# tomershay100/mp3-steganography-lib

Hardware: AMD Instinct MI355X
Metric: MP3 frames/sec (decode+re-encode) @44.1kHz stereo 128kbps, 1→8 GPU (higher is better)
Workload: dtype f64 (decode) / int32 (encode); 1 GPU; 10000-frame full decode->stego-embed->re-encode pipeline per MI355X (BASELINE configs[2]); MP3 main data + side info resident in HBM, MP3 frames out; the message cursor chain is decided and the serial chains of the rate loop are checked on the device inside every step; frames_per_gpu=10000, channels=2, message_bits=536, chain_verdict_units_to_redo=0, message_variant_entries=1874, parallelism=frames sharded over 1 GPU(s), no collective

## Files before the change

mp3-steganography-lib_amd/csrc/k_rate.hpp:

```cpp
#pragma once
#ifndef MP3S_RL_STATS
#define MP3S_RL_STATS 0
#endif
#ifndef MP3S_RL_OCC
#define MP3S_RL_OCC 6
#endif
#if MP3S_RL_STATS
__device__ unsigned long long g_rl_stats[128];
extern "C" __attribute__((visibility("default"))) int mp3s_debug_rl_stats(unsigned long long *out, int clear)
{
    (void)hipDeviceSynchronize();
    int rc = (int)hipMemcpyFromSymbol(out, HIP_SYMBOL(g_rl_stats), sizeof(unsigned long long) * 128);
    if (clear) { unsigned long long z[128] = {}; rc |= (int)hipMemcpyToSymbol(HIP_SYMBOL(g_rl_stats), z, sizeof z); }
    return rc;
}
#define RL_STAT(i, v) do { if ((threadIdx.x & 63) == 0) atomicAdd(&g_rl_stats[(i)], (unsigned long long)(v)); } while (0)
#define RL_CLK() __builtin_readcyclecounter()
#else
#define RL_STAT(i, v) do { } while (0)
#endif

namespace mp3s {

__device__ __forceinline__ uint32_t mulr_u(uint32_t a, uint32_t b) { return (uint32_t)(((uint64_t)a * b + 0x80000000ull) >> 32); }

constexpr int REDO_CAP = 4096, REDO_HEAD = 4, REDO_WORDS = REDO_HEAD + 6 * REDO_CAP;
constexpr int REDO_GROUPS = 256;
constexpr int REDO_CHAIN_MAX = 64;
constexpr int RL_WAVES = 4;
constexpr int RL_NP = 5;

struct RlTables {
    uint16_t int2idx[10000];
    uint2 hl[256];
    uint32_t c1w[16];
    uint8_t transform[64];
    uint32_t subdiv[292];
};

__device__ __forceinline__ int lin_bits_of(int t)
{
    return t < 16 ? 0 : (int)(((t < 24 ? 0xDA864321u : 0xDB987654u) >> (4 * (t & 7))) & 15u);
}

struct RlState {
    int big_values, count1, c1sel, r0c, r1c, a1, a2, a3, ts0, ts1, ts2;
    bool addr_fresh, used_addr_in;
};

__device__ __forceinline__ int family_of(int t) { return t == 13 ? 0 : (t == 15 ? 1 : (t < 24 ? 2 : 3)); }

__device__ __forceinline__ uint32_t pair_bits(const RlTables &tb, int fam, int lb, int x, int y)
{
    const int xx = x > 14 ? 15 : x, yy = y > 14 ? 15 : y;
    const uint32_t h = tb.hl[xx * 16 + yy].x;
    return ((h >> (5 * fam)) & 31u) + ((h >> 20) & 3u) + (uint32_t)lb * ((h >> 22) & 3u);
}
__device__ __forceinline__ int sel3(int r, int a, int b, int c) { return r == 0 ? a : (r == 1 ? b : c); }

__device__ __forceinline__ uint32_t rl_scale_of(int step)
{
    return (uint32_t)c_tab.steptabi[(step + 127) & 127];
}

__device__ __forceinline__ int rl_quantize(const RlTables &tb, const uint32_t (&xa)[2 * RL_NP], int32_t (&ix)[2 * RL_NP],
                                           int step, uint32_t scalei, uint32_t xrmax)
{
    const int idx = step + 127;
    if (idx < 0 || idx > 127) return -1;
    const uint32_t lnmax = mulr_u(xrmax, scalei);
    if (lnmax > 165140u) return 16384;
    if (lnmax < 10000u) {
#pragma unroll
        for (int e = 0; e < 2 * RL_NP; e++) ix[e] = tb.int2idx[mulr_u(xa[e], scalei)];
        return 0;
    }
    const double scale = c_tab.steptab[idx];
    bool big = false;
#pragma unroll
    for (int e = 0; e < 2 * RL_NP; e++) {
        uint32_t a = xa[e];
        asm volatile("" : "+v"(a));
        const uint32_t ln = mulr_u(a, scalei);
        const double dbl = (double)a * scale * 4.656612875e-10;
        const int32_t v = (int32_t)__dsqrt_rn(__dsqrt_rn(dbl) * dbl);
        ix[e] = ln >= 10000u ? v : (int32_t)tb.int2idx[ln < 10000u ? ln : 9999u];
        big |= ix[e] > 8192;
    }
    return __ballot(big) ? 8193 : 0;
}

__device__ __forceinline__ void rl_run_lengths(const RlTables &tb, int k0, int k1, RlState &st)
{
    const unsigned long long nzm = __ballot(k0 != 0), bgm = __ballot(k1 != 0);
    const int L0 = 63 - (nzm ? __builtin_clzll(nzm) : 0), L1 = 63 - (bgm ? __builtin_clzll(bgm) : 0);
    const int r0 = __builtin_amdgcn_readlane(k0, L0), r1 = __builtin_amdgcn_readlane(k1, L1);
    const int P0 = nzm ? 5 * L0 + r0 - 1 : -1, P1 = bgm ? 5 * L1 + r1 - 1 : -1;
    const int count1 = (P0 - P1) >> 1;
    const int bv = (P0 + 1) - 2 * count1;
    st.count1 = count1;
    st.big_values = bv;
    if (bv == 0) {
        st.r0c = 0; st.r1c = 0;
        if (!st.addr_fresh) st.used_addr_in = true;
    } else {
        const uint32_t e = (uint32_t)__builtin_amdgcn_readfirstlane((int)tb.subdiv[bv < 289 ? bv : 288]);
        st.r0c = (int)(e & 15); st.r1c = (int)((e >> 4) & 7);
        st.a1 = (int)((e >> 8) & 1023); st.a2 = (int)((e >> 18) & 1023);
        st.a3 = 2 * bv;
        st.addr_fresh = true;
    }
}

__device__ __forceinline__ int rl_precheck(const RlTables &tb, const uint32_t (&xa)[2 * RL_NP], int p0, RlState &st, int step, uint32_t scalei,
                                           uint32_t xrmax, int limit, bool &q_early)
{
    q_early = false;
    const int idx = step + 127;
    if (idx < 0 || idx > 127) return -1;
    if (mulr_u(xrmax, scalei) > 165140u) { q_early = true; return 100000; }
    const uint32_t t1 = (uint32_t)c_tab.rl_t1[idx], t2 = (uint32_t)c_tab.rl_t2[idx], t8 = (uint32_t)c_tab.rl_t8[idx];
    if (xrmax >= t8) return 100000;
    int k0 = 0, k1 = 0;
    uint32_t nnz = 0, nzp = 0;
#pragma unroll
    for (int m = 0; m < RL_NP; m++) {
        const uint32_t pm = max(xa[2 * m], xa[2 * m + 1]);
        k0 = pm >= t1 ? m + 1 : k0;
        k1 = pm >= t2 ? m + 1 : k1;
        nzp |= pm >= t1 ? 1u << m : 0u;
        nnz += (xa[2 * m] >= t1 ? 1u : 0u) + (xa[2 * m + 1] >= t1 ? 1u : 0u);
    }
    rl_run_lengths(tb, k0, k1, st);
    const int below = min(max(st.big_values - p0, 0), RL_NP);
    nnz += (uint32_t)__builtin_popcount(nzp & ((1u << below) - 1u));
    const int lb = (int)wave_add_u32(nnz) + st.count1;
    return lb >= limit ? lb : -1;
}

__device__ __forceinline__ int rl_body(const RlTables &tb, const int32_t (&ix)[2 * RL_NP], int p0,
                                       RlState &st, const uint8_t *__restrict__ hide, int n_hide, int cursor,
                                       int limit, bool ub_ok, bool &full)
{
    int k0 = 0, k1 = 0;
#pragma unroll
    for (int m = 0; m < RL_NP; m++) {
        const uint32_t o = (uint32_t)(ix[2 * m] | ix[2 * m + 1]);
        k0 = o != 0 ? m + 1 : k0;
        k1 = o > 1 ? m + 1 : k1;
    }
    rl_run_lengths(tb, k0, k1, st);
    const int count1 = st.count1, bv = st.big_values, bvr = 2 * bv;

    uint32_t h[RL_NP], c2[RL_NP + 1];
    uint32_t bnd = 0, acc = 0;
    {
        const int reach = st.a2 > bvr ? st.a2 : bvr;
        const int d_bv = bv - p0, d_reach = ((reach + 1) >> 1) - p0;
#pragma unroll
        for (int m = 0; m < RL_NP; m++) {
            const int x = ix[2 * m], y = ix[2 * m + 1];
            const uint2 hh = tb.hl[(x > 14 ? 15 : x) * 16 + (y > 14 ? 15 : y)];
            h[m] = hh.x;
            bnd += m < d_bv ? hh.y : (m < d_reach ? hh.y & 0xffff0000u : 0u);
        }
        if (count1 > 0) {
#pragma unroll
            for (int m = 0; m < RL_NP; m++) c2[m] = (uint32_t)(ix[2 * m] + 2 * ix[2 * m + 1]);
            c2[RL_NP] = (uint32_t)__builtin_amdgcn_update_dpp(0, (int)c2[0], 0x130, 0xf, 0xf, false);
            const uint32_t c1n = (uint32_t)(2 * count1);
            const uint32_t rel0 = (uint32_t)(p0 - bv);
            const uint32_t keep_even = (rel0 & 1u) ? 0xffff0000u : 0xffffffffu, keep_odd = (rel0 & 1u) ? 0xffffffffu : 0xffff0000u;
#pragma unroll
            for (int m = 0; m < RL_NP; m++) {
                const uint32_t quad = tb.c1w[(c2[m] | (c2[m + 1] << 2)) & 15u];
                acc += rel0 + (uint32_t)m < c1n ? quad & ((m & 1) ? keep_odd : keep_even) : 0u;
            }
            wave_add2(bnd, acc);
        } else bnd = wave_add_u32(bnd);
    }
    const int signs = (int)(acc >> 16), sum0 = signs + (int)(acc & 0xffff), sum1 = signs + 4 * count1;
    int bits;
    if (sum0 < sum1) { st.c1sel = 0; bits = sum0; } else { st.c1sel = 1; bits = sum1; }
    full = false;
    {
        const int lb = bits + (int)(bnd & 0xffffu), ub = bits + (int)(bnd >> 16);
        if (lb >= limit) return lb;
        if (ub_ok && ub < limit) return ub;
        full = true;
    }

    const int a1 = st.a1, a2 = st.a2;
    uint32_t mx0 = 0, mx1 = 0, mx2 = 0;
    int rid[RL_NP];
    const int d_a1 = ((a1 + 1) >> 1) - p0, d_a2 = ((a2 + 1) >> 1) - p0, d_bv3 = bv - p0;
#pragma unroll
    for (int m = 0; m < RL_NP; m++) {
        const uint32_t pm = (uint32_t)max(ix[2 * m], ix[2 * m + 1]);
        const bool in0 = m < d_a1, in1 = !in0 && m < d_a2, in2 = !in0 && !in1 && m < d_bv3;
        mx0 = max(mx0, in0 ? pm : 0u);
        mx1 = max(mx1, in1 ? pm : 0u);
        mx2 = max(mx2, in2 ? pm : 0u);
        rid[m] = in0 ? 0 : (in1 ? 1 : (in2 ? 2 : -1));
    }
    wave_max3(mx0, mx1, mx2);
    const int rmax[3] = {(int)mx0, (int)mx1, (int)mx2};

    int tA[3], tB[3];
    uint32_t Kr[3];
#pragma unroll
    for (int r = 0; r < 3; r++) {
        const int mxr = rmax[r];
        const int need = mxr - 15;
        const int nb = need > 0 ? 32 - __builtin_clz((unsigned)need) : 0;
        const int kA = (int)((0x77766554432100ull >> (4 * nb)) & 15ull);
        const int kB = (int)((0x77665432100000ull >> (4 * nb)) & 15ull);
        const bool none = mxr == 0, small = mxr < 15, esc0 = need == 0;
        tA[r] = none ? 0 : (small ? 13 : (esc0 ? 15 : 16 + kA));
        tB[r] = none ? 0 : (small ? 15 : 24 + kB);
        const uint32_t lbA = (0xDA864321u >> (4 * kA)) & 15u, lbB = (0xDB987654u >> (4 * kB)) & 15u;
        const uint32_t big = (esc0 ? 5u : (10u | (lbA << 16))) | (15u << 8) | (lbB << 20);
        Kr[r] = none ? (25u | (25u << 8)) : (small ? (0u | (5u << 8)) : big);
    }
#if MP3S_RL_STATS
    RL_STAT(63, 1);
    if (rmax[0] < 15 && rmax[1] < 15 && rmax[2] < 15) RL_STAT(64, 1);
    if (rmax[1] < 15 && rmax[2] < 15) RL_STAT(65, 1);
#endif
    uint32_t w0 = 0, w1 = 0, w2 = 0;
#pragma unroll
    for (int m = 0; m < RL_NP; m++) {
        const int r = rid[m];
        const uint32_t kp = (uint32_t)sel3(r, (int)Kr[0], (int)Kr[1], (int)Kr[2]);
        const uint32_t nz = __builtin_amdgcn_ubfe(h[m], 20, 2), esc = __builtin_amdgcn_ubfe(h[m], 22, 2);
        const uint32_t a = __builtin_amdgcn_ubfe(h[m], kp & 31u, 5) + nz + __builtin_amdgcn_ubfe(kp, 16, 4) * esc;
        const uint32_t b = __builtin_amdgcn_ubfe(h[m], (kp >> 8) & 31u, 5) + nz + __builtin_amdgcn_ubfe(kp, 20, 4) * esc;
        const uint32_t v = a | (b << 16);
        w0 += r == 0 ? v : 0u;
        w1 += r == 1 ? v : 0u;
        w2 += r == 2 ? v : 0u;
    }
    wave_add3(w0, w1, w2);
    const uint32_t wsum[3] = {w0, w1, w2};
    int ts[3], rbits[3];
    bool redo[3];
    int idx = cursor;
#pragma unroll
    for (int r = 0; r < 3; r++) {
        ts[r] = 0; rbits[r] = 0; redo[r] = false;
        if (tA[r]) {
            const uint32_t s = wsum[r];
            const int bA = (int)(s & 0xffff), bB = (int)(s >> 16);
            int choice;
            if (tA[r] == 13) choice = (bB <= bA) ? 15 : 13;
            else choice = (bB < bA) ? tB[r] : tA[r];
            if (n_hide > 0 && idx < n_hide) choice = tb.transform[choice * 2 + (hide[idx] & 1)];
            ts[r] = choice;
            if (choice == tA[r]) rbits[r] = bA;
            else if (choice == tB[r]) rbits[r] = bB;
            else redo[r] = true;
            if (choice > 0) idx += 1;
        }
    }
    if (redo[0] || redo[1] || redo[2]) {
        uint32_t extra = 0;
        const int f0 = family_of(ts[0]), f1 = family_of(ts[1]), f2 = family_of(ts[2]);
        const int l0 = lin_bits_of(ts[0]), l1 = lin_bits_of(ts[1]), l2 = lin_bits_of(ts[2]);
#pragma unroll
        for (int m = 0; m < RL_NP; m++) {
            const int r = rid[m];
            const bool rd = r >= 0 && sel3(r, redo[0], redo[1], redo[2]) != 0;
            const uint32_t v = pair_bits(tb, sel3(r, f0, f1, f2), sel3(r, l0, l1, l2), ix[2 * m], ix[2 * m + 1]);
            extra += rd ? v : 0u;
        }
        bits += (int)wave_add_u32(extra);
    }
    st.ts0 = ts[0]; st.ts1 = ts[1]; st.ts2 = ts[2];
    return bits + rbits[0] + rbits[1] + rbits[2];
}

struct RateVariants {
    const int32_t *unit, *cursor;
    int n;
    int16_t *ix; mp3s_gr_out *out; int32_t *en;
    uint8_t *tables;
};

template <bool CHAIN = false>
__device__ __forceinline__ void rate_units(
    const int32_t *__restrict__ mdct, const mp3s_rate_frame *__restrict__ frames, int n_units,
    const uint8_t *__restrict__ hide, int n_hide_all, const int32_t *__restrict__ cursor_in,
    const int32_t *__restrict__ state_in, const int32_t *__restrict__ unit_list, int n_list,
    int16_t *__restrict__ ix_out, mp3s_gr_out *__restrict__ out, int32_t *__restrict__ en_out, int out_base, int compact,
    RateVariants var, const int32_t *__restrict__ cursor_all = nullptr)
{
    const int n_total = n_list + var.n;
    __shared__ __attribute__((aligned(16))) RlTables tb;
#if MP3S_RL_STATS
    const unsigned long long clk0 = RL_CLK();
#endif
    const int sr0 = frames[0].sr_idx;
    const int sr_wg = sr0 >= 0 && sr0 < 3 ? sr0 : 0;
    const int wave = __builtin_amdgcn_readfirstlane(threadIdx.x >> 6), lane = threadIdx.x & 63;
    const int p0 = 5 * lane;
    int2 xpre[RL_NP];
    int u_pre = -1;
    if (!CHAIN) {
        const int li = blockIdx.x * RL_WAVES + wave;
        if (li < n_list + var.n) {
            const int32_t *ul = li >= n_list ? var.unit : unit_list;
            const int lj = li >= n_list ? li - n_list : li;
            u_pre = __builtin_amdgcn_readfirstlane(ul ? ul[lj] : lj);
            if (u_pre >= 0 && u_pre < n_units) {
                const int32_t *xr = mdct + (long)u_pre * 576;
#pragma unroll
                for (int m = 0; m < RL_NP; m++) {
                    xpre[m] = make_int2(0, 0);
                    if (p0 + m < 288) xpre[m] = *reinterpret_cast<const int2 *>(xr + 2 * (p0 + m));
                }
            }
        }
    }
    static_assert(sizeof(tb.int2idx) % 16 == 0 && sizeof(c_tab.int2idx) == sizeof(tb.int2idx), "int2idx is staged 16 bytes at a time");
    static_assert(sizeof(tb.hl) == sizeof(c_tab.rl_hl) && sizeof(tb.hl) % 1024 == 0, "the pair words are staged one wave-load (1 KB) at a time");
    static_assert(offsetof(RlTables, hl) % 16 == 0 && offsetof(RlTables, subdiv) % 16 == 0 && sizeof(tb.subdiv) % 16 == 0, "16-byte pieces in LDS");
    constexpr int I2I_CHUNKS = (int)(sizeof(tb.int2idx) / 16), I2I_ROUNDS = (I2I_CHUNKS + RL_WAVES * 64 - 1) / (RL_WAVES * 64);
    constexpr int HL_CHUNKS = (int)(sizeof(tb.hl) / 16), SD_CHUNKS = (int)(sizeof(tb.subdiv) / 16);
    static_assert(HL_CHUNKS + SD_CHUNKS <= RL_WAVES * 64 && HL_CHUNKS % 64 == 0, "pair words and region table: one piece per thread");
    uint32_t t_c1w = 0, t_tr = 0;
    {
        typedef const __attribute__((address_space(1))) void *gsrc;
        typedef __attribute__((address_space(3))) void *ldst;
        char *const lds0 = reinterpret_cast<char *>(&tb);
        const char *const g_i2i = reinterpret_cast<const char *>(c_tab.int2idx);
#pragma unroll
        for (int r = 0; r < I2I_ROUNDS; r++) {
            const int base = (r * RL_WAVES + wave) * 64;
            if (base + lane < I2I_CHUNKS)
                __builtin_amdgcn_global_load_lds((gsrc)(g_i2i + (size_t)(base + lane) * 16), (ldst)(lds0 + offsetof(RlTables, int2idx) + base * 16), 16, 0, 0);
        }
        {
            const int base = wave * 64;
            const bool is_hl = base < HL_CHUNKS;
            const char *src = is_hl ? reinterpret_cast<const char *>(c_tab.rl_hl) + (size_t)(base + lane) * 16
                                    : reinterpret_cast<const char *>(c_tab.subdiv_lut[sr_wg]) + (size_t)(base - HL_CHUNKS + lane) * 16;
            char *dst = is_hl ? lds0 + offsetof(RlTables, hl) + base * 16 : lds0 + offsetof(RlTables, subdiv) + (base - HL_CHUNKS) * 16;
            if (is_hl || base - HL_CHUNKS + lane < SD_CHUNKS) __builtin_amdgcn_global_load_lds((gsrc)src, (ldst)dst, 16, 0, 0);
        }
        if (threadIdx.x < 16) t_c1w = c_tab.rl_c1w[threadIdx.x];
        if (threadIdx.x < 64) t_tr = c_tab.transform[threadIdx.x >> 1][threadIdx.x & 1];
    }
    auto tables_in = [&]() {
        if (threadIdx.x < 16) tb.c1w[threadIdx.x] = t_c1w;
        if (threadIdx.x < 64) tb.transform[threadIdx.x] = (uint8_t)t_tr;
        __builtin_amdgcn_s_waitcnt(0);
        __syncthreads();
    };
    if (CHAIN) tables_in();

    int li0 = blockIdx.x * RL_WAVES + wave;
    if (li0 >= n_total) { if (!CHAIN) tables_in(); return; }
    do {
    int li = li0;
    uint8_t *tables_out = nullptr;
    if (li >= n_list) {
        li -= n_list;
        tables_out = var.tables;
        unit_list = var.unit; cursor_in = var.cursor; state_in = nullptr;
        ix_out = var.ix; out = var.out; en_out = var.en;
        compact = 2;
    }
    int u = CHAIN ? __builtin_amdgcn_readfirstlane(unit_list ? unit_list[li] : li) : u_pre;
    if (u < 0 || u >= n_units) { if (CHAIN) continue; tables_in(); return; }
    bool chained = false;
    int ch_cursor = 0, ch_state[4] = {0, 0, 0, 0};
    for (int steps = 0; ; steps++) {
    if (CHAIN) __builtin_amdgcn_wave_barrier();
    const mp3s_rate_frame fr = frames[u >> 2];
    const int sr = sr_wg;
    const int max_bits = fr.max_bits;
    const int ci = compact ? li : u;
    const int cursor = chained ? ch_cursor : ((n_hide_all > 0 && cursor_in) ? cursor_in[ci] : 0);
    const int n_hide = min(n_hide_all, fr.hide_end);

    const int32_t *xr = mdct + (long)u * 576;
    uint32_t xa[2 * RL_NP];
    uint32_t negmask = 0, lmax = 0, esum = 0;
    uint32_t pk[2 * RL_NP - 1];
#pragma unroll
    for (int m = 0; m < RL_NP; m++) {
        const int p = p0 + m;
        int2 v = make_int2(0, 0);
        if (!CHAIN) v = xpre[m];
        else if (p < 288) v = *reinterpret_cast<const int2 *>(xr + 2 * p);
        const int32_t vv[2] = {v.x, v.y};
#pragma unroll
        for (int e = 0; e < 2; e++) {
            const uint32_t a = vv[e] < 0 ? (0u - (uint32_t)vv[e]) : (uint32_t)vv[e];
            xa[2 * m + e] = a;
            if (vv[e] < 0) negmask |= 1u << (2 * m + e);
            lmax = max(lmax, a);
            const int32_t sq = (int32_t)(((uint64_t)a * a + (1ull << 30)) >> 31);
            const int32_t e10 = sq >> 10;
            esum += (uint32_t)e10;
            if (2 * m + e < 2 * RL_NP - 1) pk[2 * m + e] = esum;
        }
    }
    uint32_t xrmax = lmax, etot = 0;
    {
        const uint32_t incl = wave_scan_u32(esum);
        etot = (uint32_t)__builtin_amdgcn_readlane((int)incl, 63);
        xrmax = wave_max_u32(lmax);
        const int bj = c_tab.sfb_long[sr][lane < 22 ? lane : 22];
        const int qj = (bj * 6554) >> 16, rj = bj - 10 * qj;
        uint32_t S = (uint32_t)__builtin_amdgcn_ds_bpermute(qj << 2, (int)(incl - esum)), part = 0;
#pragma unroll
        for (int k = 0; k < 2 * RL_NP - 1; k++) {
            const uint32_t v = (uint32_t)__builtin_amdgcn_ds_bpermute(qj << 2, (int)pk[k]);
            part = rj == k + 1 ? v : part;
        }
        S += part;
        const uint32_t Sn = (uint32_t)__builtin_amdgcn_update_dpp(0, (int)S, 0x130, 0xf, 0xf, false);
        const int32_t temp = lane < 21 ? (int32_t)(Sn - S) : (lane == 21 ? (int32_t)etot : 0);
        int32_t en = 0;
        if (lane < 22 && temp > 0) {
            const int k = 31 - __builtin_clz((unsigned)temp);
            en = c_tab.en_base[k] + (temp >= c_tab.en_step[k] ? 1 : 0);
        }
        if (lane < 22) en_out[(long)(compact == 2 ? li : u - out_base) * 22 + lane] = en;
        RlState st;
        st.big_values = st.count1 = st.c1sel = st.r0c = st.r1c = 0;
        const int in_a1 = __builtin_amdgcn_readfirstlane(chained ? ch_state[0] : (state_in ? state_in[(long)ci * 4 + 0] : 0));
        const int in_a2 = __builtin_amdgcn_readfirstlane(chained ? ch_state[1] : (state_in ? state_in[(long)ci * 4 + 1] : 0));
        const int in_a3 = __builtin_amdgcn_readfirstlane(chained ? ch_state[2] : (state_in ? state_in[(long)ci * 4 + 2] : 0));
        const int in_given = in_a1 | (in_a2 << 10) | (in_a3 << 20);
        st.a1 = in_a1; st.a2 = in_a2; st.a3 = in_a3;
        int qstep = chained ? ch_state[3] : (state_in ? state_in[(long)ci * 4 + 3] : 0);
        st.ts0 = st.ts1 = st.ts2 = 0;
        st.addr_fresh = false; st.used_addr_in = false;
        int32_t ix[2 * RL_NP];
#pragma unroll
        for (int e = 0; e < 2 * RL_NP; e++) ix[e] = 0;
        int bits = 0, flags = 0;
        bool err = false;

#if MP3S_RL_STATS
        const unsigned long long clk1 = RL_CLK();
#endif
        if (!CHAIN) tables_in();
#if MP3S_RL_STATS
        const unsigned long long clk2 = RL_CLK();
        unsigned long long clk3 = clk2, clk4 = clk2, clk5 = clk2;
        RL_STAT(54, clk1 - clk0); RL_STAT(55, clk2 - clk1); RL_STAT(60, 1);
        int probe_j = 0;
#endif
        if (xrmax) {
            flags |= MP3S_RF_ACTIVE;
            RL_STAT(35, 1);
            int next = -120, count = 120;
            int body_step = 1 << 20, body_bits = 0;
            uint32_t sc = rl_scale_of(next + count / 2);
            asm volatile("s_mov_b32 %0, %0" : "+s"(sc));
            {
                const uint32_t sc_lo = rl_scale_of(next + 30), sc_hi = rl_scale_of(next + 90);
                bool q_early;
                const int bit = rl_precheck(tb, xa, p0, st, next + 60, sc, xrmax, max_bits, q_early);
                if (bit >= 0) {
                    if (bit < max_bits) { count = 60; sc = sc_lo; }
                    else { next += 60; count -= 60; sc = sc_hi; }
                    asm volatile("s_mov_b32 %0, %0" : "+s"(sc));
#if MP3S_RL_STATS
                    RL_STAT(0 * 5 + 0, 1); RL_STAT(40, 1); RL_STAT(47, 1); probe_j = 1;
#endif
                }
            }
#if MP3S_RL_STATS
            clk3 = RL_CLK();
#endif
            do {
                const int half = count / 2;
                const uint32_t sc_lo = rl_scale_of(next + half / 2), sc_hi = rl_scale_of(next + half + (count - half) / 2);
                const int q = rl_quantize(tb, xa, ix, next + half, sc, xrmax);
                int bit;
                if (q < 0) { err = true; break; }
                if (q > 8192) { bit = 100000; if (q != 16384) body_step = 1 << 20; RL_STAT(probe_j * 5 + 1, 1); }
                else {
                    bool full;
                    bit = rl_body(tb, ix, p0, st, hide, n_hide, cursor, max_bits, half > 1, full);
                    if (full) { body_step = next + half; body_bits = bit; } else body_step = 1 << 20;
#if MP3S_RL_STATS
                    RL_STAT(probe_j * 5 + (full ? 4 : (bit >= max_bits ? 2 : 3)), 1);
                    RL_STAT(62, 1); if (st.count1 > 0) RL_STAT(61, 1);
#endif
                }
#if MP3S_RL_STATS
                if (bit >= max_bits) {
                    RlState st2 = st; bool qe;
                    const int pb = rl_precheck(tb, xa, p0, st2, next + half, sc, xrmax, max_bits, qe);
                    RL_STAT(40 + probe_j, 1); if (pb >= max_bits) RL_STAT(47 + probe_j, 1);
                }
                probe_j++;
#endif
                if (bit < max_bits) { count = half; sc = sc_lo; }
                else { next += half; count -= half; sc = sc_hi; }
            } while (count > 1);
            qstep = next;
#if MP3S_RL_STATS
            clk4 = RL_CLK();
#endif
            if (!err) {
                if (max_bits < 0) qstep -= 1;
                do {
                    if (qstep + 1 == body_step) {
                        qstep += 1;
                        bits = body_bits;
                        body_step = 1 << 20;
                        RL_STAT(37, 1);
                        continue;
                    }
                    int q;
                    while ((q = rl_quantize(tb, xa, ix, qstep + 1, rl_scale_of(qstep + 1), xrmax)) > 8192) qstep += 1;
                    if (q < 0) { err = true; break; }
                    qstep += 1;
                    bool full;
                    bits = rl_body(tb, ix, p0, st, hide, n_hide, cursor, max_bits + 1, false, full);
#if MP3S_RL_STATS
                    RL_STAT(36, 1); RL_STAT(full ? 39 : 38, 1); RL_STAT(62, 1); if (st.count1 > 0) RL_STAT(61, 1);
#endif
                } while (bits > max_bits);
            }
            if (err) flags |= MP3S_RF_STEP_RANGE;
#if MP3S_RL_STATS
            clk5 = RL_CLK();
            RL_STAT(56, clk3 - clk2); RL_STAT(57, clk4 - clk3); RL_STAT(58, clk5 - clk4);
#endif
        }
        if (st.used_addr_in) flags |= MP3S_RF_USED_ADDR_IN;
        if (CHAIN && !chained) flags |= MP3S_RF_LISTED;

        int16_t *ixo = ix_out + (long)(compact == 2 ? li : u - out_base) * 576;
#pragma unroll
        for (int m = 0; m < RL_NP; m++) {
            const int p = p0 + m;
            if (p < 288) {
                int a = xrmax ? ix[2 * m] : 0, b = xrmax ? ix[2 * m + 1] : 0;
                if ((negmask >> (2 * m)) & 1) a = -a;
                if ((negmask >> (2 * m + 1)) & 1) b = -b;
                *reinterpret_cast<uint32_t *>(ixo + 2 * p) = ((uint32_t)(uint16_t)(int16_t)a) | ((uint32_t)(uint16_t)(int16_t)b << 16);
            }
        }
        if (lane == 0) {
            mp3s_gr_out o;
            const bool act = xrmax != 0;
            o.part2_3_length = act ? bits : 0;
            o.big_values = act ? st.big_values : 0;
            o.count1 = act ? st.count1 : 0;
            o.quantizer_step = qstep;
            o.region0_count = act ? st.r0c : 0;
            o.region1_count = act ? st.r1c : 0;
            o.count1table_select = act ? st.c1sel : 0;
            o.table_select[0] = act ? st.ts0 : 0;
            o.table_select[1] = act ? st.ts1 : 0;
            o.table_select[2] = act ? st.ts2 : 0;
            o.address[0] = st.a1; o.address[1] = st.a2; o.address[2] = st.a3;
            o.n_tables = act ? (st.ts0 > 0) + (st.ts1 > 0) + (st.ts2 > 0) : 0;
            o.flags = flags;
            o.reserved0 = (state_in || chained) ? in_given : 0;
            o.xrmax = (int32_t)xrmax;
            o.reserved = 0;
            out[compact == 1 || compact == 2 ? li : u - out_base] = o;
            if (tables_out) tables_out[li] = (uint8_t)o.n_tables;
        }
#if MP3S_RL_STATS
        RL_STAT(59, RL_CLK() - clk5);
#endif
        if (!CHAIN) break;
        ch_state[0] = __builtin_amdgcn_readfirstlane(st.a1); ch_state[1] = __builtin_amdgcn_readfirstlane(st.a2);
        ch_state[2] = __builtin_amdgcn_readfirstlane(st.a3); ch_state[3] = __builtin_amdgcn_readfirstlane(qstep);
        bool go = false;
        int un = u;
        for (;;) {
            un += 4;
            if (++steps >= REDO_CHAIN_MAX || un >= n_units || frames[un >> 2].stream != fr.stream) break;
            const int f2 = __builtin_amdgcn_readfirstlane(__hip_atomic_load(&out[un - out_base].flags, __ATOMIC_RELAXED, __HIP_MEMORY_SCOPE_AGENT));
            if (f2 & MP3S_RF_LISTED) break;
            if (!(f2 & MP3S_RF_ACTIVE)) continue;
            const int given = __builtin_amdgcn_readfirstlane(__hip_atomic_load(&out[un - out_base].reserved0, __ATOMIC_RELAXED, __HIP_MEMORY_SCOPE_AGENT));
            go = (f2 & MP3S_RF_USED_ADDR_IN) && given != (ch_state[0] | (ch_state[1] << 10) | (ch_state[2] << 20));
            break;
        }
        if (!go) break;
        u = un; chained = true;
        ch_cursor = (n_hide_all > 0 && cursor_all) ? cursor_all[u] : 0;
    }
    }
    } while (CHAIN && (li0 += (int)gridDim.x * RL_WAVES) < n_total);
}

__global__ __launch_bounds__(RL_WAVES * 64, MP3S_RL_OCC) void k_rate_loop(
    const int32_t *__restrict__ mdct, const mp3s_rate_frame *__restrict__ frames, int n_units,
    const uint8_t *__restrict__ hide, int n_hide, const int32_t *__restrict__ cursor_in,
    const int32_t *__restrict__ state_in, const int32_t *__restrict__ unit_list, int n_list,
    int16_t *__restrict__ ix_out, mp3s_gr_out *__restrict__ out, int32_t *__restrict__ en_out, int out_base, int compact,
    RateVariants var)
{
    rate_units(mdct, frames, n_units, hide, n_hide, cursor_in, state_in, unit_list, n_list, ix_out, out, en_out, out_base, compact, var);
}

__global__ __launch_bounds__(RL_WAVES * 64, 4) void k_rate_redo(
    const int32_t *__restrict__ mdct, const mp3s_rate_frame *__restrict__ frames, int n_units,
    const uint8_t *__restrict__ hide, int n_hide, const int32_t *__restrict__ redo, int16_t *__restrict__ ix_out,
    mp3s_gr_out *__restrict__ out, int32_t *__restrict__ en_out, const int32_t *__restrict__ cursor_all)
{
    const int32_t *unit_list = redo + REDO_HEAD;
    const int n_list = min(__builtin_amdgcn_readfirstlane(__hip_atomic_load(&redo[0], __ATOMIC_RELAXED, __HIP_MEMORY_SCOPE_AGENT)), REDO_CAP);
    if ((int)blockIdx.x * RL_WAVES >= n_list) return;
    const RateVariants none = {nullptr, nullptr, 0, nullptr, nullptr, nullptr, nullptr};
    rate_units<true>(mdct, frames, n_units, hide, n_hide, unit_list + REDO_CAP, unit_list + 2 * REDO_CAP, unit_list, n_list, ix_out, out, en_out,
                  0, 3, none, cursor_all);
}

__global__ __launch_bounds__(256) void k_gather_tables(const mp3s_gr_out *__restrict__ outv, int n, uint8_t *__restrict__ tables)
{
    const int i = blockIdx.x * 256 + threadIdx.x;
    if (i < n) tables[i] = (uint8_t)outv[i].n_tables;
}

__global__ __launch_bounds__(256) void k_scatter_entries(const int2 *__restrict__ pairs, int n_pairs, const int16_t *__restrict__ ixv,
                                                         const int32_t *__restrict__ env, const mp3s_gr_out *__restrict__ outv,
                                                         int16_t *__restrict__ ix, int32_t *__restrict__ en, mp3s_gr_out *__restrict__ out)
{
    const int wave = __builtin_amdgcn_readfirstlane(threadIdx.x >> 6), lane = threadIdx.x & 63;
    const int j = blockIdx.x * 4 + wave;
    if (j >= n_pairs) return;
    const int2 pr = pairs[j];
    if (pr.x < 0) return;
    const long src = pr.x, dst = pr.y;
    const uint32_t *a = reinterpret_cast<const uint32_t *>(ixv + src * 576);
    uint32_t *b = reinterpret_cast<uint32_t *>(ix + dst * 576);
    for (int i = lane; i < 288; i += 64) b[i] = a[i];
    if (lane < 22) en[dst * 22 + lane] = env[src * 22 + lane];
    static_assert(sizeof(mp3s_gr_out) % 4 == 0, "GrInfo is copied by words");
    if (lane < (int)(sizeof(mp3s_gr_out) / 4))
        reinterpret_cast<uint32_t *>(out + dst)[lane] = reinterpret_cast<const uint32_t *>(outv + src)[lane];
}

}
```

Measured before the change: 21.69 million frames/s.

## Trim rate-loop register pressure and write granule records across lanes

Several micro-changes land in the rate loop kernel. The first probe's scales and thresholds are hoisted into scalar registers before the tables are loaded. The per-element sign mask is dropped and signs are recovered by reloading the MDCT input at output time using byte-perm packing. The energy term is computed with a bitfield extract. The 72-byte output record is now built with writelane and stored as one word per lane instead of a single-lane struct store. The goal is to cut VGPR pressure and serial lane-0 store work, at the cost of a second global read of the input lines and dependence on the struct layout, which static_asserts guard.

```diff
diff --git a/mp3-steganography-lib_amd/csrc/k_rate.hpp b/mp3-steganography-lib_amd/csrc/k_rate.hpp
--- a/mp3-steganography-lib_amd/csrc/k_rate.hpp
+++ b/mp3-steganography-lib_amd/csrc/k_rate.hpp
@@ -90,7 +90,7 @@
     return __ballot(big) ? 8193 : 0;
 }
 
-__device__ __forceinline__ void rl_run_lengths(const RlTables &tb, int k0, int k1, RlState &st)
+__device__ __forceinline__ int rl_run_counts(int k0, int k1, RlState &st)
 {
     const unsigned long long nzm = __ballot(k0 != 0), bgm = __ballot(k1 != 0);
     const int L0 = 63 - (nzm ? __builtin_clzll(nzm) : 0), L1 = 63 - (bgm ? __builtin_clzll(bgm) : 0);
@@ -100,26 +100,36 @@
     const int bv = (P0 + 1) - 2 * count1;
     st.count1 = count1;
     st.big_values = bv;
-    if (bv == 0) {
-        st.r0c = 0; st.r1c = 0;
-        if (!st.addr_fresh) st.used_addr_in = true;
-    } else {
-        const uint32_t e = (uint32_t)__builtin_amdgcn_readfirstlane((int)tb.subdiv[bv < 289 ? bv : 288]);
-        st.r0c = (int)(e & 15); st.r1c = (int)((e >> 4) & 7);
-        st.a1 = (int)((e >> 8) & 1023); st.a2 = (int)((e >> 18) & 1023);
-        st.a3 = 2 * bv;
-        st.addr_fresh = true;
+    return bv;
+}
+__device__ __forceinline__ void rl_regions_none(RlState &st)
+{
+    st.r0c = 0; st.r1c = 0;
+    if (!st.addr_fresh) st.used_addr_in = true;
+}
+__device__ __forceinline__ void rl_regions(RlState &st, int bv, uint32_t e)
+{
+    st.r0c = (int)(e & 15); st.r1c = (int)((e >> 4) & 7);
+    st.a1 = (int)((e >> 8) & 1023); st.a2 = (int)((e >> 18) & 1023);
+    st.a3 = 2 * bv;
+    st.addr_fresh = true;
+}
+__device__ __forceinline__ void rl_run_lengths(const RlTables &tb, int k0, int k1, RlState &st)
+{
+    const int bv = rl_run_counts(k0, k1, st);
+    if (bv == 0) rl_regions_none(st);
+    else {
+        rl_regions(st, bv, (uint32_t)__builtin_amdgcn_readfirstlane((int)tb.subdiv[bv < 289 ? bv : 288]));
     }
 }
 
 __device__ __forceinline__ int rl_precheck(const RlTables &tb, const uint32_t (&xa)[2 * RL_NP], int p0, RlState &st, int step, uint32_t scalei,
-                                           uint32_t xrmax, int limit, bool &q_early)
+                                           uint32_t t1, uint32_t t2, uint32_t t8, uint32_t xrmax, int limit, bool &q_early)
 {
     q_early = false;
     const int idx = step + 127;
     if (idx < 0 || idx > 127) return -1;
     if (mulr_u(xrmax, scalei) > 165140u) { q_early = true; return 100000; }
-    const uint32_t t1 = (uint32_t)c_tab.rl_t1[idx], t2 = (uint32_t)c_tab.rl_t2[idx], t8 = (uint32_t)c_tab.rl_t8[idx];
     if (xrmax >= t8) return 100000;
     int k0 = 0, k1 = 0;
     uint32_t nnz = 0, nzp = 0;
@@ -131,10 +141,13 @@
         nzp |= pm >= t1 ? 1u << m : 0u;
         nnz += (xa[2 * m] >= t1 ? 1u : 0u) + (xa[2 * m + 1] >= t1 ? 1u : 0u);
     }
-    rl_run_lengths(tb, k0, k1, st);
-    const int below = min(max(st.big_values - p0, 0), RL_NP);
+    const int bv = rl_run_counts(k0, k1, st);
+    const uint32_t ev = tb.subdiv[bv < 289 ? bv : 288];
+    const int below = min(max(bv - p0, 0), RL_NP);
     nnz += (uint32_t)__builtin_popcount(nzp & ((1u << below) - 1u));
     const int lb = (int)wave_add_u32(nnz) + st.count1;
+    if (bv == 0) rl_regions_none(st);
+    else rl_regions(st, bv, (uint32_t)__builtin_amdgcn_readfirstlane((int)ev));
     return lb >= limit ? lb : -1;
 }
 
@@ -303,6 +316,9 @@
     const int sr_wg = sr0 >= 0 && sr0 < 3 ? sr0 : 0;
     const int wave = __builtin_amdgcn_readfirstlane(threadIdx.x >> 6), lane = threadIdx.x & 63;
     const int p0 = 5 * lane;
+    static_assert(-120 + 60 + 127 == 67, "the first probe's step");
+    uint32_t pre_sc = rl_scale_of(-60), pre_lo = rl_scale_of(-90), pre_hi = rl_scale_of(-30);
+    uint32_t pre_t1 = c_tab.rl_t1[67], pre_t2 = c_tab.rl_t2[67], pre_t8 = c_tab.rl_t8[67];
     int2 xpre[RL_NP];
     int u_pre = -1;
     if (!CHAIN) {
@@ -384,8 +400,15 @@
     const int n_hide = min(n_hide_all, fr.hide_end);
 
     const int32_t *xr = mdct + (long)u * 576;
+    const int32_t *xlane = xr + 2 * p0;
+    uint32_t *ixw = reinterpret_cast<uint32_t *>(ix_out + (long)(compact == 2 ? li : u - out_base) * 576) + p0;
+    int *recw = reinterpret_cast<int *>(out + (compact == 1 || compact == 2 ? li : u - out_base)) + lane;
+    asm volatile("" : "+v"(xlane), "+v"(ixw), "+v"(recw));
+    typedef int i32x2 __attribute__((ext_vector_type(2)));
+    typedef const __attribute__((address_space(1))) i32x2 *g_lines;
+    typedef __attribute__((address_space(1))) uint32_t *g_words;
     uint32_t xa[2 * RL_NP];
-    uint32_t negmask = 0, lmax = 0, esum = 0;
+    uint32_t lmax = 0, esum = 0;
     uint32_t pk[2 * RL_NP - 1];
 #pragma unroll
     for (int m = 0; m < RL_NP; m++) {
@@ -396,12 +419,11 @@
         const int32_t vv[2] = {v.x, v.y};
 #pragma unroll
         for (int e = 0; e < 2; e++) {
-            const uint32_t a = vv[e] < 0 ? (0u - (uint32_t)vv[e]) : (uint32_t)vv[e];
+            const uint32_t a = (uint32_t)max(vv[e], (int32_t)(0u - (uint32_t)vv[e]));
             xa[2 * m + e] = a;
-            if (vv[e] < 0) negmask |= 1u << (2 * m + e);
             lmax = max(lmax, a);
-            const int32_t sq = (int32_t)(((uint64_t)a * a + (1ull << 30)) >> 31);
-            const int32_t e10 = sq >> 10;
+            int32_t e10;
+            asm("v_bfe_i32 %0, %1, 9, 22" : "=v"(e10) : "v"((uint32_t)(((uint64_t)a * a + (1ull << 30)) >> 32)));
             esum += (uint32_t)e10;
             if (2 * m + e < 2 * RL_NP - 1) pk[2 * m + e] = esum;
         }
@@ -447,6 +469,7 @@
 #if MP3S_RL_STATS
         const unsigned long long clk1 = RL_CLK();
 #endif
+        asm volatile("" : "+s"(pre_sc), "+s"(pre_lo), "+s"(pre_hi), "+s"(pre_t1), "+s"(pre_t2), "+s"(pre_t8));
         if (!CHAIN) tables_in();
 #if MP3S_RL_STATS
         const unsigned long long clk2 = RL_CLK();
@@ -459,12 +482,11 @@
             RL_STAT(35, 1);
             int next = -120, count = 120;
             int body_step = 1 << 20, body_bits = 0;
-            uint32_t sc = rl_scale_of(next + count / 2);
-            asm volatile("s_mov_b32 %0, %0" : "+s"(sc));
+            uint32_t sc = pre_sc;
             {
-                const uint32_t sc_lo = rl_scale_of(next + 30), sc_hi = rl_scale_of(next + 90);
+                const uint32_t sc_lo = pre_lo, sc_hi = pre_hi;
                 bool q_early;
-                const int bit = rl_precheck(tb, xa, p0, st, next + 60, sc, xrmax, max_bits, q_early);
+                const int bit = rl_precheck(tb, xa, p0, st, next + 60, sc, pre_t1, pre_t2, pre_t8, xrmax, max_bits, q_early);
                 if (bit >= 0) {
                     if (bit < max_bits) { count = 60; sc = sc_lo; }
                     else { next += 60; count -= 60; sc = sc_hi; }
@@ -496,7 +518,8 @@
 #if MP3S_RL_STATS
                 if (bit >= max_bits) {
                     RlState st2 = st; bool qe;
-                    const int pb = rl_precheck(tb, xa, p0, st2, next + half, sc, xrmax, max_bits, qe);
+                    const int ti = (next + half + 127) & 127;
+                    const int pb = rl_precheck(tb, xa, p0, st2, next + half, sc, (uint32_t)c_tab.rl_t1[ti], (uint32_t)c_tab.rl_t2[ti], (uint32_t)c_tab.rl_t8[ti], xrmax, max_bits, qe);
                     RL_STAT(40 + probe_j, 1); if (pb >= max_bits) RL_STAT(47 + probe_j, 1);
                 }
                 probe_j++;
@@ -538,38 +561,56 @@
         if (st.used_addr_in) flags |= MP3S_RF_USED_ADDR_IN;
         if (CHAIN && !chained) flags |= MP3S_RF_LISTED;
 
-        int16_t *ixo = ix_out + (long)(compact == 2 ? li : u - out_base) * 576;
-#pragma unroll
-        for (int m = 0; m < RL_NP; m++) {
-            const int p = p0 + m;
-            if (p < 288) {
-                int a = xrmax ? ix[2 * m] : 0, b = xrmax ? ix[2 * m + 1] : 0;
-                if ((negmask >> (2 * m)) & 1) a = -a;
-                if ((negmask >> (2 * m + 1)) & 1) b = -b;
-                *reinterpret_cast<uint32_t *>(ixo + 2 * p) = ((uint32_t)(uint16_t)(int16_t)a) | ((uint32_t)(uint16_t)(int16_t)b << 16);
+        if (xrmax == 0) {
+#pragma unroll
+            for (int m = 0; m < RL_NP; m++)
+                if (p0 + m < 288) ((g_words)ixw)[m] = 0u;
+        } else {
+            typedef short s16x2 __attribute__((ext_vector_type(2)));
+            i32x2 sg[RL_NP];
+#pragma unroll
+            for (int m = 0; m < RL_NP; m++) {
+                sg[m] = i32x2{0, 0};
+                if (p0 + m < 288) sg[m] = ((g_lines)xlane)[m];
             }
-        }
-        if (lane == 0) {
-            mp3s_gr_out o;
+#pragma unroll
+            for (int m = 0; m < RL_NP; m++) {
+                const uint32_t pk = __builtin_amdgcn_perm((uint32_t)ix[2 * m + 1], (uint32_t)ix[2 * m], 0x05040100u);
+                const s16x2 top = __builtin_bit_cast(s16x2, __builtin_amdgcn_perm((uint32_t)sg[m].y, (uint32_t)sg[m].x, 0x07060302u));
+                const s16x2 neg = top >> 15;
+                const s16x2 val = __builtin_bit_cast(s16x2, pk ^ __builtin_bit_cast(uint32_t, neg)) - neg;
+                if (p0 + m < 288) ((g_words)ixw)[m] = __builtin_bit_cast(uint32_t, val);
+            }
+        }
+        {
+            static_assert(sizeof(mp3s_gr_out) == 72 && offsetof(mp3s_gr_out, part2_3_length) == 0 && offsetof(mp3s_gr_out, big_values) == 4 &&
+                          offsetof(mp3s_gr_out, count1) == 8 && offsetof(mp3s_gr_out, quantizer_step) == 12 && offsetof(mp3s_gr_out, region0_count) == 16 &&
+                          offsetof(mp3s_gr_out, region1_count) == 20 && offsetof(mp3s_gr_out, count1table_select) == 24 &&
+                          offsetof(mp3s_gr_out, table_select) == 28 && offsetof(mp3s_gr_out, address) == 40 && offsetof(mp3s_gr_out, n_tables) == 52 &&
+                          offsetof(mp3s_gr_out, flags) == 56 && offsetof(mp3s_gr_out, reserved0) == 60 && offsetof(mp3s_gr_out, xrmax) == 64 &&
+                          offsetof(mp3s_gr_out, reserved) == 68, "the record is written word by word: lane i holds word i");
             const bool act = xrmax != 0;
-            o.part2_3_length = act ? bits : 0;
-            o.big_values = act ? st.big_values : 0;
-            o.count1 = act ? st.count1 : 0;
-            o.quantizer_step = qstep;
-            o.region0_count = act ? st.r0c : 0;
-            o.region1_count = act ? st.r1c : 0;
-            o.count1table_select = act ? st.c1sel : 0;
-            o.table_select[0] = act ? st.ts0 : 0;
-            o.table_select[1] = act ? st.ts1 : 0;
-            o.table_select[2] = act ? st.ts2 : 0;
-            o.address[0] = st.a1; o.address[1] = st.a2; o.address[2] = st.a3;
-            o.n_tables = act ? (st.ts0 > 0) + (st.ts1 > 0) + (st.ts2 > 0) : 0;
-            o.flags = flags;
-            o.reserved0 = (state_in || chained) ? in_given : 0;
-            o.xrmax = (int32_t)xrmax;
-            o.reserved = 0;
-            out[compact == 1 || compact == 2 ? li : u - out_base] = o;
-            if (tables_out) tables_out[li] = (uint8_t)o.n_tables;
+            const int n_tables = act ? min(st.ts0, 1) + min(st.ts1, 1) + min(st.ts2, 1) : 0;
+            int rec = 0;
+#define RL_REC(field, k, v) asm("v_writelane_b32 %0, %1, %2" : "+v"(rec) : "s"(__builtin_amdgcn_readfirstlane((int)(v))), "n"((int)(offsetof(mp3s_gr_out, field) / 4) + (k)))
+            RL_REC(part2_3_length, 0, act ? bits : 0);
+            RL_REC(big_values, 0, act ? st.big_values : 0);
+            RL_REC(count1, 0, act ? st.count1 : 0);
+            RL_REC(quantizer_step, 0, qstep);
+            RL_REC(region0_count, 0, act ? st.r0c : 0);
+            RL_REC(region1_count, 0, act ? st.r1c : 0);
+            RL_REC(count1table_select, 0, act ? st.c1sel : 0);
+            RL_REC(table_select, 0, act ? st.ts0 : 0);
+            RL_REC(table_select, 1, act ? st.ts1 : 0);
+            RL_REC(table_select, 2, act ? st.ts2 : 0);
+            RL_REC(address, 0, st.a1); RL_REC(address, 1, st.a2); RL_REC(address, 2, st.a3);
+            RL_REC(n_tables, 0, n_tables);
+            RL_REC(flags, 0, flags);
+            RL_REC(reserved0, 0, (state_in || chained) ? in_given : 0);
+            RL_REC(xrmax, 0, xrmax);
+#undef RL_REC
+            if (lane < (int)(sizeof(mp3s_gr_out) / 4)) *(g_words)recw = (uint32_t)rec;
+            if (tables_out && lane == 0) tables_out[li] = (uint8_t)n_tables;
         }
 #if MP3S_RL_STATS
         RL_STAT(59, RL_CLK() - clk5);
```

Measured after the change: 21.65 million frames/s. No clear change (-0.2%).
